# jedward225/MARL-HideAndSeek

Hardware: AMD Instinct MI355X
Metric: world-steps/sec (agent-steps/sec derived) at 16K worlds, 1/2/4/8 GPU (higher is better)
Workload: dtype f32; 1 GPU; 16000 worlds/GPU x 2646 steps, 2 hiders + 2 seekers, sim_flags=0, rand_seed=0, random move actions in [-5,4] each step (scripts/benchmark.py args); worlds_per_gpu=16000, total_worlds=16000, agents_per_world=4

## Files before the change

### marl-hideandseek_amd/csrc/hs_k_physics.h

```cpp
#pragma once
#include "hs_state.h"
#include "hs_rays.h"
#include "hs_collide.h"
#include "hs_solver.h"
#include "hs_broadphase.h"
#include "hs_k_reset.h"

namespace hs {

constexpr int kPhysThreads = 64;
constexpr int kWorldLanes = kPhysThreads / kTile;
constexpr int kLdsWalls = 32;
static_assert(kMaxSCand <= 32 && kMaxDDCand <= 16, "accepted-manifold masks are one word per world");
constexpr int kAllDD = kNumDSlots * (kNumDSlots - 1) / 2;
constexpr int kAllSC = kNumDSlots * (kMaxWalls + kMaxPlanes - 1);
constexpr int kSpInfoWords = kNumDSlots + 1;

struct alignas(16) OctRes {
    static constexpr int kClip = kClipLanes;
    static constexpr int kClipWords = clip_words(kClip);
    static constexpr int kSatPairs = kClip < hs::kSatPairs ? kClip : hs::kSatPairs;
    static constexpr int kMaxItems = kTile * (kMaxDDCand + kMaxSCand);
    static constexpr int kSlots = kClip < 31 ? kClip : 31;
    static constexpr int kVelOffsetWords = 2 * 8 * 3 * 32;
    float pos[3][kNumDSlots][kTile];
    float rot[4][kNumDSlots][kTile];
    float ppos[3][kNumDSlots][kTile];
    float prot[4][kNumDSlots][kTile];
    int meta[kNumDSlots][kTile];
    union {
        struct {
            float lo[3][kNumDSlots][kTile], hi[3][kNumDSlots][kTile];
            float wall[4][kLdsWalls][kTile];
            unsigned xch[kNumDSlots][kTile];
        } det;
        struct {
            float clip[kClipWords];
            unsigned short items[kMaxItems + 32];
            int pend[4][kClip];
        } sat;
        struct {
            float pad[kVelOffsetWords];
            float lin[3][kNumDSlots][kTile];
            float ang[3][kNumDSlots][kTile];
        } vel;
    } u;
    unsigned short ddPair[kMaxDDCand][kTile];
    unsigned short scPair[kMaxSCand][kTile];
    unsigned short scInfo[kNumDSlots][kTile];
    unsigned int scAcc[kTile];
    unsigned int ddAcc[kTile];
    unsigned int ddOrd[2][kTile];
    float plane0[4][kTile];
    unsigned char bodies[kNumDSlots * kTile];
    union {
        unsigned char wallBodies[kNumDSlots * kTile];
        unsigned char actGL[kMaxAgents][kTile];
    };
    unsigned int wallSeen[kTile];
    unsigned char numWalls[kTile], numPlanes[kTile], ndd[kTile], nsc[kTile], seen[kTile], hasGrab[kTile];
    unsigned char spill[kTile];
    int wid[kTile];
};
constexpr int kSeenDeferred = 2;
static_assert(sizeof(OctRes) <= 20 * 1024, "8 waves of 8 worlds share the CU's 160 KiB of LDS");
static_assert(offsetof(OctRes, u.sat.items) >= offsetof(OctRes, u.det.wall), "items must not overlap the AABBs");
static_assert(sizeof(decltype(OctRes::u.det)) <= sizeof(decltype(OctRes::u.sat)), "the broadphase scratch adds nothing to the octet's LDS");
static_assert(sizeof(ManDD) / 4 * OctRes::kSlots <= OctRes::kVelOffsetWords, "manifold slots lie below the velocities");
static_assert(2 * 3 * kNumDSlots * 8 <= OctRes::kVelOffsetWords, "the hull AABBs lie below the velocities");

constexpr int kLocGlobal = 31;
HSD int pair_a(int p) { return p & 31; }
HSD int pair_b(int p) { return (p >> 5) & 63; }
HSD int pair_loc(int p) { return (p >> 11) & 31; }
HSD int pair_pack(int a, int b) { return a | (b << 5) | (kLocGlobal << 11); }
static_assert(kNumDSlots <= 32 && kMaxWalls + kMaxPlanes <= 64, "pair encoding");
static_assert(sizeof(ManDD) % 16 == 0 && sizeof(ManS) % 16 == 0, "manifold records move 16 bytes at a time");
constexpr int kManWords = sizeof(ManDD) / 4;
template <typename M> HSD void man_lds_load(const float *clip, int slot, M &m) {
    m = *reinterpret_cast<const M *>(clip + slot * kManWords);
}
template <typename M> HSD void man_lds_set_lam(float *clip, int slot, int j, float v) {
    static_assert(offsetof(M, lam) == sizeof(M) - 16, "lam is the record's tail");
    clip[slot * kManWords + (sizeof(M) / 4 - 4 + j)] = v;
}

template <int C> HSD V3 rld3(const float (&a)[C][kNumDSlots][kTile], int slot, int g) { return {a[0][slot][g], a[1][slot][g], a[2][slot][g]}; }
HSD Q rld4(const float (&a)[4][kNumDSlots][kTile], int slot, int g) { return {a[0][slot][g], a[1][slot][g], a[2][slot][g], a[3][slot][g]}; }
HSD void rst3(float (&a)[3][kNumDSlots][kTile], int slot, int g, V3 v) { a[0][slot][g] = v.x; a[1][slot][g] = v.y; a[2][slot][g] = v.z; }
HSD void rst4(float (&a)[4][kNumDSlots][kTile], int slot, int g, Q q) { a[0][slot][g] = q.w; a[1][slot][g] = q.x; a[2][slot][g] = q.y; a[3][slot][g] = q.z; }

HSD void rbody_load(const OctRes &R, int g, int slot, BodyS &b) {
    b.pos = rld3(R.pos, slot, g); b.rot = rld4(R.rot, slot, g);
    b.ppos = rld3(R.ppos, slot, g); b.prot = rld4(R.prot, slot, g);
    b.lin = rld3(R.u.vel.lin, slot, g); b.ang = rld3(R.u.vel.ang, slot, g);
    const int m = R.meta[slot][g];
    const bool dyn = m != 0 && meta_resp(m) == RESP_DYNAMIC;
    b.invM = dyn ? obj_inv_mass(meta_obj(m)) : 0.f;
    b.invI = dyn ? obj_inv_inertia(meta_obj(m)) : V3{0.f, 0.f, 0.f};
    body_refresh_inertia(b);
}
HSD void rbody_store_pose(OctRes &R, int g, int slot, const BodyS &b) { rst3(R.pos, slot, g, b.pos); rst4(R.rot, slot, g, b.rot); }
HSD void rbody_store_vel(OctRes &R, int g, int slot, const BodyS &b) { rst3(R.u.vel.lin, slot, g, b.lin); rst3(R.u.vel.ang, slot, g, b.ang); }
HSD void derive_velocity(BodyS &b) {
    const float h = kSubstepH;
    b.lin = (b.pos - b.ppos) * (1.f / h);
    Q dq = qmul(b.rot, qinv(b.prot));
    V3 wv = V3{dq.x, dq.y, dq.z} * (2.f / h);
    b.ang = dq.w >= 0.f ? wv : -wv;
}

HSD void wave_sync() { asm volatile("s_waitcnt lgkmcnt(0)" ::: "memory"); }
HSD void mem_sync() { asm volatile("s_waitcnt vmcnt(0) lgkmcnt(0)" ::: "memory"); }

template <int D> HSD int dpp_row_shr(int x) { return __builtin_amdgcn_update_dpp(0, x, 0x110 + D, 0xF, 0xF, true); }
HSD int scan8_incl(int x, int l) {
    int y;
// ... 334 lines not shown
    if (l == 0) {
        R.spill[g] = (unsigned char)((spillDD ? 1 : 0) | (spillSC ? 2 : 0));
        if (spillDD || spillSC) spInfo[0] = tot_dd | (tot_sc << 16);
        R.ndd[g] = (unsigned char)min(tot_dd, kMaxDDCand); R.nsc[g] = (unsigned char)min(tot_sc, kMaxSCand);
        if (R.wid[g] >= 0 && tot_dd + tot_sc > 0) S.loadAcc[R.wid[g]] += tot_dd + tot_sc;
    }
    wave_sync();
    return ic;
}

template <bool POS, int UNROLL, typename SetLam>
HSD void static_manifold(BodyS &me, const ManS &m, SetLam set_lam) {
    BodyS none;
    body_refresh_inertia(me);
    const V3 n = ld3(m.n);
    const int np = m.np;
    const float mu = POS ? m.muS : m.muD;
#pragma unroll UNROLL
    for (int j = 0; j < 4; ++j)
        if (j < np) {
            const float lamj = m.lam[j];
            if (POS) set_lam(j, lamj + solve_point_position<false>(me, none, n, ld3(m.rA[j]), V3{0.f, 0.f, 0.f}, m.offB[j], mu));
            else solve_point_velocity<false>(me, none, n, ld3(m.rA[j]), V3{0.f, 0.f, 0.f}, lamj, mu);
        }
}

#define HS_COLD __device__ __forceinline__
struct SpillCtx {
    const float *walls, *planes;
    ManDD *wsDD; ManS *wsSC; unsigned short *spPair; int *spInfo;
    int wbeg;
};
HSD SpillCtx spill_ctx(const SimState &S) { return {S.walls.p, S.planes.p, (ManDD *)S.wsDD, (ManS *)S.wsSC, S.spPair, S.spInfo, S.wbeg}; }

HS_COLD void spill_sat(SpillCtx c, OctRes *Rp) {
    OctRes &R = *Rp;
    const int lane = hs_lane() & 63;
    const bool hi = (lane & 1) != 0;
    const Col<float, 4 * kMaxWalls> walls = {const_cast<float *>(c.walls)};
    const Col<float, 4 * kMaxPlanes> planes = {const_cast<float *>(c.planes)};
#pragma unroll 1
    for (int g = 0; g < kTile; ++g) {
        const int fl = __builtin_amdgcn_readfirstlane((int)R.spill[g]);
        if (fl == 0) continue;
        const int w = c.wbeg + g;
        const int tot = __builtin_amdgcn_readfirstlane(c.spInfo[(size_t)w * kSpInfoWords]);
#pragma unroll 1
        for (int kind = 0; kind < 2; ++kind) {
            if ((fl & (1 << kind)) == 0) continue;
            const bool isdd = kind == 0;
            const int n = isdd ? tot & 0xffff : tot >> 16;
#pragma unroll 1
            for (int base = isdd ? kMaxDDCand : kMaxSCand; base < n; base += OctRes::kSatPairs) {
                const int kk = base + (lane >> 1);
                if (kk < n && (lane >> 1) < OctRes::kSatPairs) {
                    const int pair = c.spPair[(size_t)w * (kAllDD + kAllSC) + (isdd ? 0 : kAllDD) + kk];
                    const int a = pair_a(pair), bsel = pair_b(pair);
                    const int oa = meta_obj(R.meta[a][g]);
                    const V3 pa = rld3(R.pos, a, g);
                    const Q qa = rld4(R.rot, a, g);
                    ManDD *const md = c.wsDD + (size_t)w * kAllDD + kk;
                    ManS *const ms = c.wsSC + (size_t)w * kAllSC + kk;
                    RawManifold raw;
                    raw.np = 0;
                    bool plane = false;
                    if (!isdd && bsel >= kMaxWalls) {
                        const int p = bsel - kMaxWalls;
                        const V3 pn = {planes(0 * kMaxPlanes + p, w), planes(1 * kMaxPlanes + p, w), planes(2 * kMaxPlanes + p, w)};
                        plane = true;
                        if (!hi && !collide_hull_plane(hull_ref_body(oa, pa, qa), pn, planes(3 * kMaxPlanes + p, w), raw)) raw.np = 0;
                    } else {
                        const HullSrc ha = hull_src_body(oa, pa, qa);
                        const HullSrc hb = isdd ? hull_src_body(meta_obj(R.meta[bsel][g]), rld3(R.pos, bsel, g), rld4(R.rot, bsel, g))
                                                : hull_src_wall(walls(0 * kMaxWalls + bsel, w), walls(1 * kMaxWalls + bsel, w),
                                                                walls(2 * kMaxWalls + bsel, w), walls(3 * kMaxWalls + bsel, w));
                        const AxisResult res = sat_axes(ha, hb, hi);
                        const ClipBuf cb = {R.u.sat.clip, lane >> 1, OctRes::kClip};
                        if (!hi && res.code != 0 && !sat_contact(ha, hb, res, cb, raw)) raw.np = 0;
                    }
                    if (!hi) {
                        const int ob = isdd ? meta_obj(R.meta[bsel][g]) : plane ? OBJ_PLANE : OBJ_WALL;
                        const float muS = 0.5f * (obj_mu_s(oa) + obj_mu_s(ob)), muD = 0.5f * (obj_mu_d(oa) + obj_mu_d(ob));
                        const Q qai = qinv(qa);
                        if (isdd) {
                            md->a = a; md->b = bsel; md->np = raw.np; md->muS = muS; md->muD = muD;
                            st3(md->n, raw.n);
                            const V3 pb = rld3(R.pos, bsel, g);
                            const Q qbi = qinv(rld4(R.rot, bsel, g));
#pragma unroll
                            for (int j = 0; j < 4; ++j)
                                if (j < raw.np) {
                                    st3(md->rA[j], qrot(qai, raw.pA[j] - pa)); st3(md->rB[j], qrot(qbi, raw.pB[j] - pb));
                                    md->lam[j] = 0.f;
                                }
                        } else {
                            ms->np = raw.np; ms->muS = muS; ms->muD = muD;
                            st3(ms->n, raw.n);
#pragma unroll
                            for (int j = 0; j < 4; ++j)
                                if (j < raw.np) {
                                    st3(ms->rA[j], plane ? hull_local_vertex(oa, raw.vidx[j]) : qrot(qai, raw.pA[j] - pa));
                                    ms->offB[j] = dot(raw.pB[j], raw.n); ms->lam[j] = 0.f;
                                }
                        }
                    }
                }
                wave_sync();
            }
// ... 30 lines not shown
                if (POS) { rbody_store_pose(R, g, ba, Ab); rbody_store_pose(R, g, bb, Bb); }
                else { rbody_store_vel(R, g, ba, Ab); rbody_store_vel(R, g, bb, Bb); }
                wave_sync();
            }
        }
    }
}

template <bool POS>
HS_COLD void spill_static(SpillCtx c, OctRes *Rp, int NS) {
    OctRes &R = *Rp;
#pragma unroll 1
    for (int g = 0; g < kTile; ++g) {
        if ((__builtin_amdgcn_readfirstlane((int)R.spill[g]) & 2) == 0) continue;
        const int w = c.wbeg + g;
        const int slot = hs_lane();
        if (slot >= NS) continue;
        const int info = c.spInfo[(size_t)w * kSpInfoWords + 1 + slot];
        const int first = info & 0xffff, cnt = info >> 16;
        if (cnt == 0) continue;
        BodyS me;
        rbody_load(R, g, slot, me);
#pragma unroll 1
        for (int k = first; k < first + cnt; ++k) {
            ManS &m = c.wsSC[(size_t)w * kAllSC + k];
            if (m.np <= 0) continue;
            static_manifold<POS, 1>(me, m, [&](int j, float v) { m.lam[j] = v; });
        }
        if (POS) rbody_store_pose(R, g, slot, me); else rbody_store_vel(R, g, slot, me);
    }
}

HSD HullSrc sat_hull_a(const OctRes &R, int g, int a) { return hull_src_body(meta_obj(R.meta[a][g]), rld3(R.pos, a, g), rld4(R.rot, a, g)); }
HSD HullSrc sat_hull_b(const SimState &S, const OctRes &R, int g, int w, bool isdd, int bsel) {
    if (isdd) return hull_src_body(meta_obj(R.meta[bsel][g]), rld3(R.pos, bsel, g), rld4(R.rot, bsel, g));
    return hull_src_wall(S.walls(0 * kMaxWalls + bsel, w), S.walls(1 * kMaxWalls + bsel, w),
                         S.walls(2 * kMaxWalls + bsel, w), S.walls(3 * kMaxWalls + bsel, w));
}
HSD bool sat_flush(const SimState &S, OctRes &R, int npend, bool last) {
    const int lane = hs_lane() & 63;
    const bool toLds = last && lane < OctRes::kSlots;
    bool wroteGlobal = false;
    int mw[kManWords]; int mkind = 0, mkk = 0, mg = 0, mpair = 0;
    if (lane < npend) {
        const int item = R.u.sat.pend[0][lane] & 0xffff;
        AxisResult res;
        res.code = R.u.sat.pend[0][lane] >> 16;
        res.ax = {__int_as_float(R.u.sat.pend[1][lane]), __int_as_float(R.u.sat.pend[2][lane]), __int_as_float(R.u.sat.pend[3][lane])};
        const int g = item >> 6, idx = item & 63;
        const int w = S.wbeg + g;
        const bool isdd = idx < 32;
        const int kk = idx & 31;
        const int pair = isdd ? R.ddPair[kk][g] : R.scPair[kk][g];
        const int a = pair_a(pair), bsel = pair_b(pair);
        const ClipBuf cb = {R.u.sat.clip, lane, OctRes::kClip};
        RawManifold raw;
        const bool plane = res.code == 3;
        bool have;
        if (plane) {
            const int p = bsel - kMaxWalls;
            const V3 pn = {S.planes(0 * kMaxPlanes + p, w), S.planes(1 * kMaxPlanes + p, w), S.planes(2 * kMaxPlanes + p, w)};
            have = collide_hull_plane(hull_ref_body(meta_obj(R.meta[a][g]), rld3(R.pos, a, g), rld4(R.rot, a, g)), pn, S.planes(3 * kMaxPlanes + p, w), raw);
        } else {
            have = sat_contact(sat_hull_a(R, g, a), sat_hull_b(S, R, g, w, isdd, bsel), res, cb, raw);
        }
        if (have) {
            const int oa = meta_obj(R.meta[a][g]);
            const int ob = isdd ? meta_obj(R.meta[bsel][g]) : plane ? OBJ_PLANE : OBJ_WALL;
            const V3 pa = rld3(R.pos, a, g);
            const Q qai = qinv(rld4(R.rot, a, g));
            const float muS = 0.5f * (obj_mu_s(oa) + obj_mu_s(ob)), muD = 0.5f * (obj_mu_d(oa) + obj_mu_d(ob));
            if (isdd) {
                ManDD m;
                m.a = a; m.b = bsel; m.np = raw.np; m.muS = muS; m.muD = muD;
                st3(m.n, raw.n);
                const V3 pb = rld3(R.pos, bsel, g);
                const Q qbi = qinv(rld4(R.rot, bsel, g));
#pragma unroll
                for (int j = 0; j < 4; ++j) {
                    const bool on = j < raw.np;
                    st3(m.rA[j], on ? qrot(qai, raw.pA[j] - pa) : V3{0.f, 0.f, 0.f});
                    st3(m.rB[j], on ? qrot(qbi, raw.pB[j] - pb) : V3{0.f, 0.f, 0.f});
                    m.lam[j] = 0.f;
                }
                if (toLds) { __builtin_memcpy(mw, &m, sizeof(m)); mkind = 1; mkk = kk; mg = g; mpair = pair; }
                else { ((ManDD *)S.wsDD + (size_t)w * kAllDD)[kk] = m; wroteGlobal = true; }
                atomicOr(&R.ddAcc[g], 1u << kk);
            } else {
                ManS m;
                m.np = raw.np; m.muS = muS; m.muD = muD; m.pad[0] = 0.f; m.pad[1] = 0.f;
                st3(m.n, raw.n);
#pragma unroll
                for (int j = 0; j < 4; ++j) {
                    const bool on = j < raw.np;
                    st3(m.rA[j], !on ? V3{0.f, 0.f, 0.f} : plane ? hull_local_vertex(oa, raw.vidx[j]) : qrot(qai, raw.pA[j] - pa));
                    m.offB[j] = on ? dot(raw.pB[j], raw.n) : 0.f; m.lam[j] = 0.f;
                }
// ... 22 lines not shown
HSD bool phase_sat(const SimState &S, OctRes &R, ItemCounts ic) {
    const int wedge0 = (ic.nbox + 31) / 32 * 32;
    const int lane = hs_lane() & 63;
    const bool hi = (lane & 1) != 0;
    int npend = 0;
    bool usedGlobal = false;
    const int boxRounds = (ic.nbox + OctRes::kSatPairs - 1) / OctRes::kSatPairs, wedgeRounds = (ic.nwedge + 3) / 4;
    if (__builtin_expect(ic.anySpill, 0)) { spill_sat(spill_ctx(S), &R); usedGlobal = true; }
    const int totalRounds = boxRounds + wedgeRounds;
    int round = 0;
    while (round < totalRounds) {
    for (; round < totalRounds; ++round) {
        const bool wide = round >= boxRounds;
        {
            const int itemsHere = wide ? min(4, wedge0 + ic.nwedge - (wedge0 + (round - boxRounds) * 4)) : min(OctRes::kSatPairs, ic.nbox - round * OctRes::kSatPairs);
            if (npend + itemsHere > OctRes::kClip) break;
        }
        const int base = wide ? wedge0 + (round - boxRounds) * 4 : round * OctRes::kSatPairs;
        const int it = wide ? base + (lane >> 4) : base + (lane >> 1);
        const bool lead = wide ? (lane & 15) == 0 : !hi;
        AxisResult res = {0, {0.f, 0.f, 0.f}};
        int item = 0;
        if (wide ? it < wedge0 + ic.nwedge : (it < ic.nbox && (lane >> 1) < OctRes::kSatPairs)) {
            item = R.u.sat.items[it];
            const int g = item >> 6, idx = item & 63;
            const int w = S.wbeg + g;
            const bool isdd = idx < 32;
            const int kk = idx & 31;
            const int pair = isdd ? R.ddPair[kk][g] : R.scPair[kk][g];
            const int a = pair_a(pair), bsel = pair_b(pair);
            if (!isdd && bsel >= kMaxWalls) {
                if (lead) res.code = 3;
            } else if (wide) {
                res = sat_axes_wide(sat_hull_a(R, g, a), sat_hull_b(S, R, g, w, isdd, bsel), lane & 15);
            } else {
                res = sat_axes(sat_hull_a(R, g, a), sat_hull_b(S, R, g, w, isdd, bsel), hi);
            }
        }
        const bool hit = lead && res.code != 0;
        const unsigned long long m = __ballot(hit);
        const int nhit = __popcll(m);
        if (hit) {
            const int pos = npend + __popcll(m & ((1ull << lane) - 1ull));
            R.u.sat.pend[0][pos] = item | (res.code << 16);
            R.u.sat.pend[1][pos] = __float_as_int(res.ax.x); R.u.sat.pend[2][pos] = __float_as_int(res.ax.y); R.u.sat.pend[3][pos] = __float_as_int(res.ax.z);
        }
        npend += nhit;
    }
    wave_sync();
    if (npend > 0) { usedGlobal |= sat_flush(S, R, npend, round >= totalRounds); npend = 0; }
    }
    if (usedGlobal) mem_sync();
    return usedGlobal;
}

HSD void solve_grab_joint_bodies(BodyS &A, BodyS &B, V3 r2, Q attach2, float sep, V3 r1, Q attach1) {
    {
        Q qa = qmul(A.rot, attach1), qb = qmul(B.rot, attach2);
        Q dq = qmul(qa, qinv(qb));
        V3 dphi = {2.f * dq.x, 2.f * dq.y, 2.f * dq.z};
        if (dq.w < 0.f) dphi = -dphi;
        float th2 = len2(dphi);
        if (th2 > 1e-12f) {
            float th = sqrtf(th2);
            V3 ax = dphi * (1.f / th);
            float wA = dot(ax, sym_mul(A.Iw, ax));
            float wB = dot(ax, sym_mul(B.Iw, ax));
            float ws = wA + wB;
            if (ws > 0.f) {
// ... 65 lines not shown
HSD void pair_point_velocity(BodyS &me, bool isA, V3 n, V3 rl, float lamN, float muD) {
    if (!(lamN > 0.f)) return;
    const V3 rw = qrot(me.rot, rl);
    const bool hm = me.invM + me.invI.x + me.invI.y + me.invI.z != 0.f;
    const V3 vm = cross_add(me.ang, rw, me.lin);
    const V3 vo = swap1(vm);
    const bool ho = swap1(hm ? 1.f : 0.f) != 0.f;
    const V3 vA = isA ? vm : vo, vB = isA ? vo : vm;
    const bool hA = isA ? hm : ho, hB = isA ? ho : hm;
    V3 v = {0.f, 0.f, 0.f};
    if (hA) v = vA;
    if (hB) v = v - vB;
    const float vn = dot(n, v);
    const V3 vt = nmadd(v, n, vn);
    const float vt2 = len2(vt);
    V3 dv = -(n * vn);
    if (vt2 > 1e-18f) {
        const float vtl = sqrtf(vt2);
        const float mag = fminf((muD * lamN) * kInvSubstepH, vtl);
        dv = nmadd(dv, vt, mag / vtl);
    }
    const float dv2 = len2(dv);
    if (!(dv2 > 1e-18f)) return;
    const float wm = gen_inv_mass_sq(me, rw, dv, dv2);
    const float wo = swap1(wm);
    const float ws = isA ? wm + wo : wo + wm;
    if (!(ws > 0.f)) return;
    const V3 p = dv * (dv2 / ws);
    const V3 da = apply_inv_inertia(me, cross(rw, p));
    if (isA) { me.lin = madd(me.lin, p, me.invM); me.ang = me.ang + da; }
    else { me.lin = nmadd(me.lin, p, me.invM); me.ang = me.ang - da; }
}

template <bool POS>
HSD void phase_dd(const SimState &S, OctRes &R, bool anySpill) {
    constexpr int GL = kWorldLanes, PAIRS = GL / 2;
    const int L = hs_lane(), g = L / GL, q = L % GL;
    const int h = q >> 1;
    const bool isA = (q & 1) == 0;
    const int gbit0 = g * GL;
    const int w = S.wbeg + g;
    const int ndd = R.ndd[g];
    const bool grab = R.hasGrab[g] != 0;
    if (!anySpill && __ballot(R.ddAcc[g] != 0u || (POS && grab)) == 0ull) return;
    if (POS && grab && q == 0) {
        const int teams = S.teams[R.wid[g]];
        for (int a = 0; a < kMaxAgents; ++a) {
            if (!team_agent_active(teams, a)) continue;
            const int other = S.grabOther(a, w);
            if (other < 0) continue;
            BodyS A, B;
            rbody_load(R, g, kAgentSlot0 + a, A); rbody_load(R, g, other, B);
            float gd[kGrabWords];
#pragma unroll
            for (int c = 0; c < kGrabWords; ++c) gd[c] = S.grabData(c * kMaxAgents + a, w);
            solve_grab_joint_bodies(A, B, {gd[0], gd[1], gd[2]}, {gd[3], gd[4], gd[5], gd[6]}, gd[7],
                                    {gd[8], gd[9], gd[10]}, {gd[11], gd[12], gd[13], gd[14]});
            rbody_store_pose(R, g, kAgentSlot0 + a, A); rbody_store_pose(R, g, other, B);
        }
    }
    ManDD *const wsDD = (ManDD *)S.wsDD + (size_t)w * kAllDD;
    const unsigned acc = R.ddAcc[g];
    const int nacc = __popc(acc);
    if (POS) {
        if (q < 2) R.ddOrd[q][g] = 0u;
        int key0 = 0x7fffffff, key1 = 0x7fffffff;
        if (q < ndd && ((acc >> q) & 1u)) { const int p = R.ddPair[q][g]; key0 = (pair_a(p) << 8) | pair_b(p); }
        if (q + GL < ndd && ((acc >> (q + GL)) & 1u)) { const int p = R.ddPair[q + GL][g]; key1 = (pair_a(p) << 8) | pair_b(p); }
        int rank0 = 0, rank1 = 0;
#pragma unroll
        for (int p = 0; p < GL; ++p) {
            const int k0 = __shfl(key0, gbit0 + p), k1 = __shfl(key1, gbit0 + p);
            rank0 += (k0 < key0) + (k1 < key0); rank1 += (k0 < key1) + (k1 < key1);
        }
        wave_sync();
        if (key0 != 0x7fffffff) atomicOr(&R.ddOrd[rank0 >> 3][g], (unsigned)q << ((rank0 & 7) * 4));
        if (key1 != 0x7fffffff) atomicOr(&R.ddOrd[rank1 >> 3][g], (unsigned)(q + GL) << ((rank1 & 7) * 4));
    }
    wave_sync();
    for (int base = 0; base < kMaxDDCand; base += PAIRS) {
        if (__ballot(base < nacc) == 0ull) break;
        const int rk = base + h;
        const int mine = rk < nacc ? (int)((R.ddOrd[rk >> 3][g] >> ((rk & 7) * 4)) & 15u) : -1;
        int ma = -1, mb = -1, loc = kLocGlobal;
        ManDD m;
        if (mine >= 0) {
            const int pr = R.ddPair[mine][g];
            ma = pair_a(pr); mb = pair_b(pr); loc = pair_loc(pr);
            if (loc != kLocGlobal) man_lds_load(R.u.sat.clip, loc, m); else m = wsDD[mine];
        }
        unsigned dep = 0u;
#pragma unroll
        for (int p = 0; p < PAIRS - 1; ++p) {
            const int pa = __shfl(ma, gbit0 + 2 * p), pb = __shfl(mb, gbit0 + 2 * p);
            if (p < h && pa >= 0 && (pa == ma || pa == mb || pb == ma || pb == mb)) dep |= 1u << p;
        }
        bool pending = mine >= 0;
        BodyS me;
        const int myBody = isA ? ma : mb;
        const V3 n = ld3(m.n);
        while (true) {
            const unsigned long long pend_mask = __ballot(pending && isA);
            if (pend_mask == 0ull) break;
            const unsigned wp = (unsigned)(pend_mask >> gbit0);
            unsigned pendPairs = 0u;
#pragma unroll
            for (int p = 0; p < PAIRS; ++p) pendPairs |= ((wp >> (2 * p)) & 1u) << p;
            if (pending && (dep & pendPairs) == 0u) {
                rbody_load(R, g, myBody, me);
                if (POS) {
#pragma unroll
                    for (int j = 0; j < 4; ++j)
                        if (j < m.np) {
                            const float lam = pair_point_position(me, isA, n, isA ? ld3(m.rA[j]) : ld3(m.rB[j]), m.muS);
                            if (isA) { if (loc != kLocGlobal) man_lds_set_lam<ManDD>(R.u.sat.clip, loc, j, m.lam[j] + lam); else wsDD[mine].lam[j] = m.lam[j] + lam; }
                        }
                    rbody_store_pose(R, g, myBody, me);
                } else {
#pragma unroll
                    for (int j = 0; j < 4; ++j)
                        if (j < m.np) pair_point_velocity(me, isA, n, isA ? ld3(m.rA[j]) : ld3(m.rB[j]), m.lam[j], m.muD);
                    rbody_store_vel(R, g, myBody, me);
                }
                pending = false;
            }
            wave_sync();
        }
    }
    wave_sync();
    if (__builtin_expect(anySpill, 0)) { spill_dd<POS>(spill_ctx(S), &R); wave_sync(); }
}

struct WallLists { int nwb, nEarly; };
template <int ROUNDS>
HSD WallLists list_wall_bodies(OctRes &R, int nbodies, int lastRound) {
    const int L = hs_lane();
    int n = 0, nEarly = 0;
#pragma unroll
    for (int r = 0; r < ROUNDS; ++r) {
        if (r == lastRound) nEarly = n;
        const bool valid = r * 64 + L < nbodies;
        const int t = valid ? R.bodies[r * 64 + L] : 0;
        const int sci = valid ? R.scInfo[t >> 3][t & 7] : 0;
        const bool on = sci != 0 && ((R.scAcc[t & 7] >> (sci & 0xff)) & ((1u << (sci >> 8)) - 1u)) != 0u;
        const unsigned long long m = __ballot(on);
        if (on) { R.wallBodies[n + __popcll(m & ((1ull << L) - 1ull))] = (unsigned char)t; atomicOr(&R.wallSeen[t & 7], 1u << (t >> 3)); }
        n += __popcll(m);
    }
    wave_sync();
    return {n, nEarly};
}

HSD void ground_pos(OctRes &R, BodyReg &b, int slot, int g, int meta) {
    if (meta_resp(meta) != RESP_DYNAMIC || b.np == 0) return;
    const int obj = meta_obj(meta);
    BodyS me;
    rbody_load(R, g, slot, me);
    const V3 gn = -V3{R.plane0[0][g], R.plane0[1][g], R.plane0[2][g]};
    const float gmuS = 0.5f * (obj_mu_s(obj) + obj_mu_s(OBJ_PLANE));
    const bool yaw = slot >= kAgentSlot0;
    float dj[4] = {0.f, 0.f, 0.f, 0.f}, share = 0.f;
    if (yaw) share = yaw_ground_prepass(me, gn, b.np, hull_local_vertex(obj, b.vidx & 7), hull_local_vertex(obj, (b.vidx >> 3) & 7),
                                        hull_local_vertex(obj, (b.vidx >> 6) & 7), hull_local_vertex(obj, (b.vidx >> 9) & 7), kGroundOff, dj);
// ... 4 lines not shown
    rbody_store_pose(R, g, slot, me);
}
HSD void ground_vel(OctRes &R, const BodyReg &b, int slot, int g, int meta) {
    if (meta_resp(meta) != RESP_DYNAMIC || b.np == 0) return;
    const int obj = meta_obj(meta);
    BodyS me, none;
    rbody_load(R, g, slot, me);
    const V3 gn = -V3{R.plane0[0][g], R.plane0[1][g], R.plane0[2][g]};
    const float gmuD = 0.5f * (obj_mu_d(obj) + obj_mu_d(OBJ_PLANE));
#pragma unroll
    for (int j = 0; j < 4; ++j)
        if (j < b.np) solve_point_velocity<false>(me, none, gn, hull_local_vertex(obj, (b.vidx >> (3 * j)) & 7), V3{0.f, 0.f, 0.f},
                                                  b.lam[j], gmuD);
    rbody_store_vel(R, g, slot, me);
}
template <bool POS>
HSD void wall_round(const SimState &S, OctRes &R, int first, int nwb) {
    for (int i = first + hs_lane(); i < nwb; i += 64) {
        const int t = R.wallBodies[i];
        const int slot = t >> 3, g = t & 7;
        const int sci = R.scInfo[slot][g];
        const int bsc = sci & 0xff, asc = sci >> 8;
        const unsigned acc = R.scAcc[g];
        ManS *const wsSC = (ManS *)S.wsSC + (size_t)(S.wbeg + g) * kAllSC;
        BodyS me;
        rbody_load(R, g, slot, me);
        unsigned todo = (acc >> bsc) & ((1u << asc) - 1u);
#pragma unroll 1
        while (todo != 0u) {
            const int k = bsc + __ffs((int)todo) - 1;
            todo &= todo - 1u;
            const int loc = pair_loc(R.scPair[k][g]);
            ManS m;
            if (loc != kLocGlobal) man_lds_load(R.u.sat.clip, loc, m); else m = wsSC[k];
            static_manifold<POS, 4>(me, m, [&](int j, float v) {
                if (loc != kLocGlobal) man_lds_set_lam<ManS>(R.u.sat.clip, loc, j, v); else wsSC[k].lam[j] = v;
            });
        }
        if (POS) rbody_store_pose(R, g, slot, me); else rbody_store_vel(R, g, slot, me);
    }
}
template <bool POS>
HSD void last_round(const SimState &S, OctRes &R, BodyReg &b, bool valid, int slot, int g, int meta, int nLast, int nMerged) {
    const int mi = (int)hs_lane() - nLast;
    const bool walls = mi >= 0 && mi < nMerged;
    unsigned todo = 0u; int bsc = 0;
    if (walls) {
        const int t = R.wallBodies[mi];
        slot = t >> 3; g = t & 7; meta = R.meta[slot][g];
        const int sci = R.scInfo[slot][g];
        bsc = sci & 0xff;
        todo = (R.scAcc[g] >> bsc) & ((1u << (sci >> 8)) - 1u);
    } else if (valid && meta_resp(meta) == RESP_DYNAMIC && b.np != 0) {
        todo = 1u;
    }
    if (todo == 0u) return;
    const int obj = meta_obj(meta);
    BodyS me, none;
    rbody_load(R, g, slot, me);
    ManS *const wsSC = (ManS *)S.wsSC + (size_t)(S.wbeg + g) * kAllSC;
#pragma unroll 1
    while (todo != 0u) {
        const int k = bsc + __ffs((int)todo) - 1;
        todo &= todo - 1u;
        V3 n; float mu; int np, loc = kLocGlobal;
        ManS m;
        if (walls) {
            loc = pair_loc(R.scPair[k][g]);
            if (loc != kLocGlobal) man_lds_load(R.u.sat.clip, loc, m); else m = wsSC[k];
            n = ld3(m.n); mu = POS ? m.muS : m.muD; np = m.np;
        } else {
            n = -V3{R.plane0[0][g], R.plane0[1][g], R.plane0[2][g]};
            mu = POS ? 0.5f * (obj_mu_s(obj) + obj_mu_s(OBJ_PLANE)) : 0.5f * (obj_mu_d(obj) + obj_mu_d(OBJ_PLANE));
            np = b.np;
        }
        body_refresh_inertia(me);
        const bool yaw = POS && !walls && slot >= kAgentSlot0;
        float dj[4] = {0.f, 0.f, 0.f, 0.f}, share = 0.f;
        if (yaw) share = yaw_ground_prepass(me, n, np, hull_local_vertex(obj, b.vidx & 7), hull_local_vertex(obj, (b.vidx >> 3) & 7),
                                            hull_local_vertex(obj, (b.vidx >> 6) & 7), hull_local_vertex(obj, (b.vidx >> 9) & 7), kGroundOff, dj);
#define HS_LAST_POINT(j)                                                                                                   \
        if ((j) < np) {                                                                                                    \
            const V3 rAj = walls ? ld3(m.rA[j]) : hull_local_vertex(obj, (b.vidx >> (3 * (j))) & 7);                       \
            const float lamj = walls ? m.lam[j] : b.lam[j];                                                                \
            if (POS) {                                                                                                     \
                const float nl = lamj + solve_point_position_ground(me, n, rAj, walls ? m.offB[j] : kGroundOff, mu, yaw, dj[j], share); \
                if (!walls) b.lam[j] = nl;                                                                                 \
                else if (loc != kLocGlobal) man_lds_set_lam<ManS>(R.u.sat.clip, loc, (j), nl);                             \
                else wsSC[k].lam[j] = nl;                                                                                  \
            } else {                                                                                                       \
                solve_point_velocity<false>(me, none, n, rAj, V3{0.f, 0.f, 0.f}, lamj, mu);                                \
            }                                                                                                              \
        }
        HS_LAST_POINT(0) HS_LAST_POINT(1) HS_LAST_POINT(2) HS_LAST_POINT(3)
#undef HS_LAST_POINT
    }
    if (POS) rbody_store_pose(R, g, slot, me); else rbody_store_vel(R, g, slot, me);
}
HSD void derive_body_velocity(OctRes &R, int slot, int g, int meta) {
    if (meta_resp(meta) != RESP_DYNAMIC) return;
    BodyS me;
    me.pos = rld3(R.pos, slot, g); me.rot = rld4(R.rot, slot, g);
    me.ppos = rld3(R.ppos, slot, g); me.prot = rld4(R.prot, slot, g);
    derive_velocity(me);
    rbody_store_vel(R, g, slot, me);
}

HSD void action_system(const SimState &S, OctRes &R, int g, int A_, int teams) {
    const int w = S.wbeg + g;
    const ResGeom geom = {R, S, g, w};
    for (int i = 0; i < A_; ++i) {
        const int fl = R.actGL[i][g];
        if (fl == 0) continue;
        const int type = team_agent_type(teams, i);
        const int slot = kAgentSlot0 + i;
        const V3 mpos = geom.g_pos(slot);
        const Q mrot = geom.g_rot(slot);
        if (fl & 2) {
            float t; V3 o = mpos + V3{0.f, 0.f, 0.5f};
            int hit = trace_ray(geom, o, qrot(mrot, {0.f, 1.f, 0.f}), 2.5f, &t);
            if (hit >= 0 && hit < kNumDSlots) {
                const int m = R.meta[hit][g];
                const int obj = meta_obj(m), resp = meta_resp(m), owner = meta_owner(m);
                if (resp == RESP_STATIC) {
                    if ((type == AGENT_SEEKER && owner == OWNER_SEEKER) || (type == AGENT_HIDER && owner == OWNER_HIDER))
                        R.meta[hit][g] = meta_pack(obj, RESP_DYNAMIC, OWNER_NONE);
                } else if (owner == OWNER_NONE) {
                    R.meta[hit][g] = meta_pack(obj, RESP_STATIC, type == AGENT_HIDER ? OWNER_HIDER : OWNER_SEEKER);
// ... 151 lines not shown
    const int L = hs_lane();
#pragma unroll
    for (int r = 0; r < LASTR; ++r) {
        const bool valid = r * 64 + L < nbodies; const int t_ = valid ? R.bodies[r * 64 + L] : 0;
        const int slot = t_ >> 3, g = t_ & 7; const int meta = valid ? R.meta[slot][g] : 0;
        if (valid) { if (POS) ground_pos(R, br[r], slot, g, meta); else ground_vel(R, br[r], slot, g, meta); }
    }
    wave_sync();
    {
        const bool valid = LASTR * 64 + L < nbodies; const int t_ = valid ? R.bodies[LASTR * 64 + L] : 0;
        const int slot = t_ >> 3, g = t_ & 7; const int meta = valid ? R.meta[slot][g] : 0;
        last_round<POS>(S, R, br[LASTR], valid, slot, g, meta, nLast, nMerged);
    }
    wave_sync();
}

#ifdef HS_PHASE_TIMING
#define HS_TICK_PARAMS , long long &tk, long long (&acc)[10]
#define HS_TICK_ARGS , tk, acc
#define HS_TICK(i) { const long long now_ = wall_clock64(); acc[i] += now_ - tk; tk = now_; }
#else
#define HS_TICK_PARAMS
#define HS_TICK_ARGS
#define HS_TICK(i)
#endif
#define HS_BODY(r) const bool valid = (r) * 64 + L < nbodies; const int t_ = valid ? R.bodies[(r) * 64 + L] : 0; \
                   const int slot = t_ >> 3, g = t_ & 7; const int meta = valid ? R.meta[slot][g] : 0;
template <int ROUNDS>
HSD void substep_rest(const SimState &S, OctRes &R, BodyReg (&br)[ROUNDS], int nbodies, int NS, ItemCounts ic, bool integrateNext,
                      const float *aforce HS_TICK_PARAMS) {
    const int L = hs_lane();
    const bool manGlobal = phase_sat(S, R, ic);
    HS_TICK(3)
    phase_dd<true>(S, R, ic.anySpill);
    HS_TICK(4)
    constexpr int kShortLastR = ROUNDS - 2;
    const bool shortLast = ROUNDS == 3 && nbodies <= 64 * (ROUNDS - 1);
    const int lastRound = shortLast ? kShortLastR : ROUNDS - 1;
    const WallLists wl = list_wall_bodies<ROUNDS>(R, nbodies, lastRound);
    const int nLast = max(nbodies - 64 * lastRound, 0);
    const int nMerged = min(wl.nEarly, 64 - nLast);
    if (shortLast) static_passes<ROUNDS, kShortLastR, true>(S, R, br, nbodies, nLast, nMerged);
    else static_passes<ROUNDS, ROUNDS - 1, true>(S, R, br, nbodies, nLast, nMerged);
    if (wl.nwb > nMerged) { wall_round<true>(S, R, nMerged, wl.nwb); wave_sync(); }
    if (__builtin_expect(ic.anySpill, 0)) { spill_static<true>(spill_ctx(S), &R, NS); wave_sync(); }
#pragma unroll
    for (int r = 0; r < ROUNDS; ++r) { HS_BODY(r) if (valid) derive_body_velocity(R, slot, g, meta); }
    if (manGlobal) mem_sync(); else wave_sync();
    HS_TICK(5)
    phase_dd<false>(S, R, ic.anySpill);
    HS_TICK(6)
    if (shortLast) static_passes<ROUNDS, kShortLastR, false>(S, R, br, nbodies, nLast, nMerged);
    else static_passes<ROUNDS, ROUNDS - 1, false>(S, R, br, nbodies, nLast, nMerged);
    if (wl.nwb > nMerged) { wall_round<false>(S, R, nMerged, wl.nwb); wave_sync(); }
    if (__builtin_expect(ic.anySpill, 0)) { spill_static<false>(spill_ctx(S), &R, NS); wave_sync(); }
    if (integrateNext) {
#pragma unroll
        for (int r = 0; r < ROUNDS; ++r) { HS_BODY(r) if (valid) integrate_body(R, br[r], slot, g, meta, aforce); }
        wave_sync();
    }
    HS_TICK(7)
}

template <int ROUNDS>
HSD void physics_step(SimState &S, OctRes &R, GenScratch *gen) {
    const int L = hs_lane();
    const int noct = gridDim.x;
    const int sidx = step_ring(S), prevIdx = sidx == 0 ? 2 : sidx - 1, nextIdx = sidx == 2 ? 0 : sidx + 1;
    const int serve = step_serve(S);
    if (serve != kGroupEarly && blockIdx.x == 0 && L == 0) {
        S.tickSum[nextIdx] = 0ull;
        atomicExch(group_count(S, prevIdx, kGroupEarly), 0); atomicExch(group_count(S, prevIdx, kGroupLate), 0);
    }
    int o = blockIdx.x;
    if (serve != kGroupAll) {
        if (o >= *group_count(S, sidx, serve)) return;
        o = oct_list(S, sidx, serve, noct)[o];
    }
    S.wbeg = o * kTile;
    const int p0 = S.wbeg;
    const int NS = kAgentSlot0 + S.A;
    const long long tStart = wall_clock64();
    int prevTicks, lateAbove;
// ... 117 lines not shown
```

Measured before the change: 35.20 million world-steps/s.

## Carry body-pair solve order in registers and load only each side's manifold pieces

```diff
diff --git a/marl-hideandseek_amd/csrc/hs_k_physics.h b/marl-hideandseek_amd/csrc/hs_k_physics.h
--- a/marl-hideandseek_amd/csrc/hs_k_physics.h
+++ b/marl-hideandseek_amd/csrc/hs_k_physics.h
@@ -4,6 +4,7 @@
 #include "hs_collide.h"
 #include "hs_solver.h"
 #include "hs_broadphase.h"
+#include "hs_solve_order.h"
 #include "hs_k_reset.h"
 
 namespace hs {
@@ -50,7 +51,6 @@
     unsigned short scInfo[kNumDSlots][kTile];
     unsigned int scAcc[kTile];
     unsigned int ddAcc[kTile];
-    unsigned int ddOrd[2][kTile];
     float plane0[4][kTile];
     unsigned char bodies[kNumDSlots * kTile];
     union {
@@ -77,12 +77,31 @@
 static_assert(kNumDSlots <= 32 && kMaxWalls + kMaxPlanes <= 64, "pair encoding");
 static_assert(sizeof(ManDD) % 16 == 0 && sizeof(ManS) % 16 == 0, "manifold records move 16 bytes at a time");
 constexpr int kManWords = sizeof(ManDD) / 4;
-template <typename M> HSD void man_lds_load(const float *clip, int slot, M &m) {
-    m = *reinterpret_cast<const M *>(clip + slot * kManWords);
-}
-template <typename M> HSD void man_lds_set_lam(float *clip, int slot, int j, float v) {
+typedef float Piece __attribute__((ext_vector_type(4)));
+#define HS_LDS __attribute__((address_space(3)))
+#define HS_GLOBAL __attribute__((address_space(1)))
+HSD Piece lds_piece(const float *p) { return *(const HS_LDS Piece *)p; }
+HSD Piece glb_piece(const float *p) { return *(const HS_GLOBAL Piece *)p; }
+HSD void lds_put_piece(float *p, Piece v) { *(HS_LDS Piece *)p = v; }
+HSD void glb_put_piece(float *p, Piece v) { *(HS_GLOBAL Piece *)p = v; }
+HSD float glb_word(const float *p) { return *(const HS_GLOBAL float *)p; }
+template <int N> struct Pieces { Piece p[N]; };
+template <int N> HSD void man_load(const float *clip, int loc, const float *rec, const int (&at)[N], Pieces<N> &out) {
+    const float *s = clip + min(loc, OctRes::kSlots - 1) * kManWords;
+#pragma unroll
+    for (int i = 0; i < N; ++i) out.p[i] = lds_piece(s + at[i]);
+    if (loc == kLocGlobal) {
+#pragma unroll
+        for (int i = 0; i < N; ++i) out.p[i] = glb_piece(rec + at[i]);
+    }
+}
+template <typename M> HSD void man_put_lam(float *clip, int loc, M *rec, Piece lam) {
     static_assert(offsetof(M, lam) == sizeof(M) - 16, "lam is the record's tail");
-    clip[slot * kManWords + (sizeof(M) / 4 - 4 + j)] = v;
+    if (loc != kLocGlobal) lds_put_piece(clip + loc * kManWords + (sizeof(M) / 4 - 4), lam);
+    else glb_put_piece(rec->lam, lam);
+}
+HSD void man_static_load(const float *clip, int loc, const ManS *rec, ManS &m) {
+    if (loc != kLocGlobal) m = *reinterpret_cast<const ManS *>(clip + loc * kManWords); else m = *rec;
 }
 
 template <int C> HSD V3 rld3(const float (&a)[C][kNumDSlots][kTile], int slot, int g) { return {a[0][slot][g], a[1][slot][g], a[2][slot][g]}; }
@@ -483,6 +502,7 @@
     int wbeg;
 };
 HSD SpillCtx spill_ctx(const SimState &S) { return {S.walls.p, S.planes.p, (ManDD *)S.wsDD, (ManS *)S.wsSC, S.spPair, S.spInfo, S.wbeg}; }
+HSD HullSrc sat_hull_b(const Col<float, 4 * kMaxWalls> &walls, const OctRes &R, int g, int w, bool isdd, int bsel);
 
 HS_COLD void spill_sat(SpillCtx c, OctRes *Rp) {
     OctRes &R = *Rp;
@@ -522,9 +542,7 @@
                         if (!hi && !collide_hull_plane(hull_ref_body(oa, pa, qa), pn, planes(3 * kMaxPlanes + p, w), raw)) raw.np = 0;
                     } else {
                         const HullSrc ha = hull_src_body(oa, pa, qa);
-                        const HullSrc hb = isdd ? hull_src_body(meta_obj(R.meta[bsel][g]), rld3(R.pos, bsel, g), rld4(R.rot, bsel, g))
-                                                : hull_src_wall(walls(0 * kMaxWalls + bsel, w), walls(1 * kMaxWalls + bsel, w),
-                                                                walls(2 * kMaxWalls + bsel, w), walls(3 * kMaxWalls + bsel, w));
+                        const HullSrc hb = sat_hull_b(walls, R, g, w, isdd, bsel);
                         const AxisResult res = sat_axes(ha, hb, hi);
                         const ClipBuf cb = {R.u.sat.clip, lane >> 1, OctRes::kClip};
                         if (!hi && res.code != 0 && !sat_contact(ha, hb, res, cb, raw)) raw.np = 0;
@@ -621,10 +639,14 @@
 }
 
 HSD HullSrc sat_hull_a(const OctRes &R, int g, int a) { return hull_src_body(meta_obj(R.meta[a][g]), rld3(R.pos, a, g), rld4(R.rot, a, g)); }
-HSD HullSrc sat_hull_b(const SimState &S, const OctRes &R, int g, int w, bool isdd, int bsel) {
-    if (isdd) return hull_src_body(meta_obj(R.meta[bsel][g]), rld3(R.pos, bsel, g), rld4(R.rot, bsel, g));
-    return hull_src_wall(S.walls(0 * kMaxWalls + bsel, w), S.walls(1 * kMaxWalls + bsel, w),
-                         S.walls(2 * kMaxWalls + bsel, w), S.walls(3 * kMaxWalls + bsel, w));
+HSD HullSrc sat_hull_b(const Col<float, 4 * kMaxWalls> &walls, const OctRes &R, int g, int w, bool isdd, int bsel) {
+    static_assert(kNumDSlots <= kMaxWalls, "a body slot is a valid wall row");
+    const float *const wp = &walls(min(bsel, kMaxWalls - 1), w);
+    const float cx = glb_word(wp), cy = glb_word(wp + kMaxWalls * kTile);
+    const float hx = glb_word(wp + 2 * kMaxWalls * kTile), hy = glb_word(wp + 3 * kMaxWalls * kTile);
+    const int slot = isdd ? bsel : 0;
+    const HullSrc body = hull_src_body(meta_obj(R.meta[slot][g]), rld3(R.pos, slot, g), rld4(R.rot, slot, g));
+    return hull_src_sel(isdd, body, hull_src_wall(cx, cy, hx, hy));
 }
 HSD bool sat_flush(const SimState &S, OctRes &R, int npend, bool last) {
     const int lane = hs_lane() & 63;
@@ -651,7 +673,7 @@
             const V3 pn = {S.planes(0 * kMaxPlanes + p, w), S.planes(1 * kMaxPlanes + p, w), S.planes(2 * kMaxPlanes + p, w)};
             have = collide_hull_plane(hull_ref_body(meta_obj(R.meta[a][g]), rld3(R.pos, a, g), rld4(R.rot, a, g)), pn, S.planes(3 * kMaxPlanes + p, w), raw);
         } else {
-            have = sat_contact(sat_hull_a(R, g, a), sat_hull_b(S, R, g, w, isdd, bsel), res, cb, raw);
+            have = sat_contact(sat_hull_a(R, g, a), sat_hull_b(S.walls, R, g, w, isdd, bsel), res, cb, raw);
         }
         if (have) {
             const int oa = meta_obj(R.meta[a][g]);
@@ -740,9 +762,9 @@
             if (!isdd && bsel >= kMaxWalls) {
                 if (lead) res.code = 3;
             } else if (wide) {
-                res = sat_axes_wide(sat_hull_a(R, g, a), sat_hull_b(S, R, g, w, isdd, bsel), lane & 15);
+                res = sat_axes_wide(sat_hull_a(R, g, a), sat_hull_b(S.walls, R, g, w, isdd, bsel), lane & 15);
             } else {
-                res = sat_axes(sat_hull_a(R, g, a), sat_hull_b(S, R, g, w, isdd, bsel), hi);
+                res = sat_axes(sat_hull_a(R, g, a), sat_hull_b(S.walls, R, g, w, isdd, bsel), hi);
             }
         }
         const bool hit = lead && res.code != 0;
@@ -874,17 +896,32 @@
     else { me.lin = nmadd(me.lin, p, me.invM); me.ang = me.ang - da; }
 }
 
+struct ManSide { int np; float muS, muD; V3 n; V3 r[4]; Piece lam; };
+HSD void man_side_load(const float *clip, int loc, const ManDD *rec, bool isA, ManSide &m) {
+    static_assert(offsetof(ManDD, rA) == 32 && offsetof(ManDD, rB) == 80 && offsetof(ManDD, lam) == 128, "pieces of a ManDD");
+    const int r0 = isA ? 8 : 20;
+    const int at[6] = {0, 4, r0, r0 + 4, r0 + 8, 32};
+    Pieces<6> q;
+    man_load(clip, loc, reinterpret_cast<const float *>(rec), at, q);
+    m.np = __float_as_int(q.p[0].z); m.muS = q.p[0].w; m.muD = q.p[1].x;
+    m.n = {q.p[1].y, q.p[1].z, q.p[1].w};
+    m.r[0] = {q.p[2].x, q.p[2].y, q.p[2].z}; m.r[1] = {q.p[2].w, q.p[3].x, q.p[3].y};
+    m.r[2] = {q.p[3].z, q.p[3].w, q.p[4].x}; m.r[3] = {q.p[4].y, q.p[4].z, q.p[4].w};
+    m.lam = q.p[5];
+}
+
 template <bool POS>
-HSD void phase_dd(const SimState &S, OctRes &R, bool anySpill) {
+HSD unsigned phase_dd(const SimState &S, OctRes &R, bool anySpill, unsigned ordIn) {
     constexpr int GL = kWorldLanes, PAIRS = GL / 2;
+    static_assert(PAIRS == kOrdBatch && kMaxDDCand <= kOrdBatch * kOrdBatches, "the order word holds every batch");
     const int L = hs_lane(), g = L / GL, q = L % GL;
     const int h = q >> 1;
     const bool isA = (q & 1) == 0;
     const int gbit0 = g * GL;
     const int w = S.wbeg + g;
-    const int ndd = R.ndd[g];
     const bool grab = R.hasGrab[g] != 0;
-    if (!anySpill && __ballot(R.ddAcc[g] != 0u || (POS && grab)) == 0ull) return;
+    const unsigned acc = R.ddAcc[g];
+    if (!anySpill && __ballot(acc != 0u || (POS && grab)) == 0ull) return 0u;
     if (POS && grab && q == 0) {
         const int teams = S.teams[R.wid[g]];
         for (int a = 0; a < kMaxAgents; ++a) {
@@ -902,66 +939,47 @@
         }
     }
     ManDD *const wsDD = (ManDD *)S.wsDD + (size_t)w * kAllDD;
-    const unsigned acc = R.ddAcc[g];
     const int nacc = __popc(acc);
-    if (POS) {
-        if (q < 2) R.ddOrd[q][g] = 0u;
-        int key0 = 0x7fffffff, key1 = 0x7fffffff;
-        if (q < ndd && ((acc >> q) & 1u)) { const int p = R.ddPair[q][g]; key0 = (pair_a(p) << 8) | pair_b(p); }
-        if (q + GL < ndd && ((acc >> (q + GL)) & 1u)) { const int p = R.ddPair[q + GL][g]; key1 = (pair_a(p) << 8) | pair_b(p); }
-        int rank0 = 0, rank1 = 0;
-#pragma unroll
-        for (int p = 0; p < GL; ++p) {
-            const int k0 = __shfl(key0, gbit0 + p), k1 = __shfl(key1, gbit0 + p);
-            rank0 += (k0 < key0) + (k1 < key0); rank1 += (k0 < key1) + (k1 < key1);
-        }
-        wave_sync();
-        if (key0 != 0x7fffffff) atomicOr(&R.ddOrd[rank0 >> 3][g], (unsigned)q << ((rank0 & 7) * 4));
-        if (key1 != 0x7fffffff) atomicOr(&R.ddOrd[rank1 >> 3][g], (unsigned)(q + GL) << ((rank1 & 7) * 4));
-    }
-    wave_sync();
-    for (int base = 0; base < kMaxDDCand; base += PAIRS) {
+    unsigned ord = POS ? 0u : ordIn;
+    wave_sync();
+    for (int base = 0, batch = 0; base < kMaxDDCand; base += PAIRS, ++batch) {
         if (__ballot(base < nacc) == 0ull) break;
         const int rk = base + h;
-        const int mine = rk < nacc ? (int)((R.ddOrd[rk >> 3][g] >> ((rk & 7) * 4)) & 15u) : -1;
-        int ma = -1, mb = -1, loc = kLocGlobal;
-        ManDD m;
+        const int mine = POS ? (rk < nacc ? kth_set_bit(acc, rk) : -1) : ord_cand(ord, batch);
+        int code = -1, loc = kLocGlobal;
+        ManSide m;
         if (mine >= 0) {
             const int pr = R.ddPair[mine][g];
-            ma = pair_a(pr); mb = pair_b(pr); loc = pair_loc(pr);
-            if (loc != kLocGlobal) man_lds_load(R.u.sat.clip, loc, m); else m = wsDD[mine];
-        }
-        unsigned dep = 0u;
-#pragma unroll
-        for (int p = 0; p < PAIRS - 1; ++p) {
-            const int pa = __shfl(ma, gbit0 + 2 * p), pb = __shfl(mb, gbit0 + 2 * p);
-            if (p < h && pa >= 0 && (pa == ma || pa == mb || pb == ma || pb == mb)) dep |= 1u << p;
-        }
+            code = pr & 0x7ff; loc = pair_loc(pr);
+            man_side_load(R.u.sat.clip, loc, wsDD + mine, isA, m);
+        }
+        unsigned dep;
+        if (POS) {
+            dep = batch_dep_mask(h, code, dpp_row_shr<2>(code), dpp_row_shr<4>(code), dpp_row_shr<6>(code));
+            if (mine >= 0) ord |= ord_pack(batch, mine, dep);
+        } else {
+            dep = ord_dep(ord, batch);
+        }
+        const unsigned depBits = dep_spread(dep);
         bool pending = mine >= 0;
         BodyS me;
-        const int myBody = isA ? ma : mb;
-        const V3 n = ld3(m.n);
+        const int myBody = isA ? pair_a(code) : pair_b(code);
         while (true) {
             const unsigned long long pend_mask = __ballot(pending && isA);
             if (pend_mask == 0ull) break;
-            const unsigned wp = (unsigned)(pend_mask >> gbit0);
-            unsigned pendPairs = 0u;
-#pragma unroll
-            for (int p = 0; p < PAIRS; ++p) pendPairs |= ((wp >> (2 * p)) & 1u) << p;
-            if (pending && (dep & pendPairs) == 0u) {
+            if (pending && (depBits & (unsigned)(pend_mask >> gbit0)) == 0u) {
                 rbody_load(R, g, myBody, me);
                 if (POS) {
+                    Piece lam = m.lam;
 #pragma unroll
                     for (int j = 0; j < 4; ++j)
-                        if (j < m.np) {
-                            const float lam = pair_point_position(me, isA, n, isA ? ld3(m.rA[j]) : ld3(m.rB[j]), m.muS);
-                            if (isA) { if (loc != kLocGlobal) man_lds_set_lam<ManDD>(R.u.sat.clip, loc, j, m.lam[j] + lam); else wsDD[mine].lam[j] = m.lam[j] + lam; }
-                        }
+                        if (j < m.np) lam[j] = lam[j] + pair_point_position(me, isA, m.n, m.r[j], m.muS);
+                    if (isA) man_put_lam(R.u.sat.clip, loc, wsDD + mine, lam);
                     rbody_store_pose(R, g, myBody, me);
                 } else {
 #pragma unroll
                     for (int j = 0; j < 4; ++j)
-                        if (j < m.np) pair_point_velocity(me, isA, n, isA ? ld3(m.rA[j]) : ld3(m.rB[j]), m.lam[j], m.muD);
+                        if (j < m.np) pair_point_velocity(me, isA, m.n, m.r[j], m.lam[j], m.muD);
                     rbody_store_vel(R, g, myBody, me);
                 }
                 pending = false;
@@ -971,6 +989,7 @@
     }
     wave_sync();
     if (__builtin_expect(anySpill, 0)) { spill_dd<POS>(spill_ctx(S), &R); wave_sync(); }
+    return ord;
 }
 
 struct WallLists { int nwb, nEarly; };
@@ -1041,10 +1060,10 @@
             todo &= todo - 1u;
             const int loc = pair_loc(R.scPair[k][g]);
             ManS m;
-            if (loc != kLocGlobal) man_lds_load(R.u.sat.clip, loc, m); else m = wsSC[k];
-            static_manifold<POS, 4>(me, m, [&](int j, float v) {
-                if (loc != kLocGlobal) man_lds_set_lam<ManS>(R.u.sat.clip, loc, j, v); else wsSC[k].lam[j] = v;
-            });
+            man_static_load(R.u.sat.clip, loc, wsSC + k, m);
+            Piece lam = {m.lam[0], m.lam[1], m.lam[2], m.lam[3]};
+            static_manifold<POS, 4>(me, m, [&](int j, float v) { lam[j] = v; });
+            if (POS) man_put_lam(R.u.sat.clip, loc, wsSC + k, lam);
         }
         if (POS) rbody_store_pose(R, g, slot, me); else rbody_store_vel(R, g, slot, me);
     }
@@ -1076,7 +1095,7 @@
         ManS m;
         if (walls) {
             loc = pair_loc(R.scPair[k][g]);
-            if (loc != kLocGlobal) man_lds_load(R.u.sat.clip, loc, m); else m = wsSC[k];
+            man_static_load(R.u.sat.clip, loc, wsSC + k, m);
             n = ld3(m.n); mu = POS ? m.muS : m.muD; np = m.np;
         } else {
             n = -V3{R.plane0[0][g], R.plane0[1][g], R.plane0[2][g]};
@@ -1094,15 +1113,14 @@
             const float lamj = walls ? m.lam[j] : b.lam[j];                                                                \
             if (POS) {                                                                                                     \
                 const float nl = lamj + solve_point_position_ground(me, n, rAj, walls ? m.offB[j] : kGroundOff, mu, yaw, dj[j], share); \
-                if (!walls) b.lam[j] = nl;                                                                                 \
-                else if (loc != kLocGlobal) man_lds_set_lam<ManS>(R.u.sat.clip, loc, (j), nl);                             \
-                else wsSC[k].lam[j] = nl;                                                                                  \
+                if (!walls) b.lam[j] = nl; else m.lam[j] = nl;                                                             \
             } else {                                                                                                       \
                 solve_point_velocity<false>(me, none, n, rAj, V3{0.f, 0.f, 0.f}, lamj, mu);                                \
             }                                                                                                              \
         }
         HS_LAST_POINT(0) HS_LAST_POINT(1) HS_LAST_POINT(2) HS_LAST_POINT(3)
 #undef HS_LAST_POINT
+        if (POS && walls) man_put_lam(R.u.sat.clip, loc, wsSC + k, Piece{m.lam[0], m.lam[1], m.lam[2], m.lam[3]});
     }
     if (POS) rbody_store_pose(R, g, slot, me); else rbody_store_vel(R, g, slot, me);
 }
@@ -1320,7 +1338,7 @@
     const int L = hs_lane();
     const bool manGlobal = phase_sat(S, R, ic);
     HS_TICK(3)
-    phase_dd<true>(S, R, ic.anySpill);
+    const unsigned ddOrder = phase_dd<true>(S, R, ic.anySpill, 0u);
     HS_TICK(4)
     constexpr int kShortLastR = ROUNDS - 2;
     const bool shortLast = ROUNDS == 3 && nbodies <= 64 * (ROUNDS - 1);
@@ -1336,7 +1354,7 @@
     for (int r = 0; r < ROUNDS; ++r) { HS_BODY(r) if (valid) derive_body_velocity(R, slot, g, meta); }
     if (manGlobal) mem_sync(); else wave_sync();
     HS_TICK(5)
-    phase_dd<false>(S, R, ic.anySpill);
+    phase_dd<false>(S, R, ic.anySpill, ddOrder);
     HS_TICK(6)
     if (shortLast) static_passes<ROUNDS, kShortLastR, false>(S, R, br, nbodies, nLast, nMerged);
     else static_passes<ROUNDS, ROUNDS - 1, false>(S, R, br, nbodies, nLast, nMerged);
diff --git a/marl-hideandseek_amd/csrc/hs_solve_order.h b/marl-hideandseek_amd/csrc/hs_solve_order.h
--- /dev/null
+++ b/marl-hideandseek_amd/csrc/hs_solve_order.h
@@ -0,0 +1,40 @@
+#pragma once
+#include "hs_core.h"
+
+namespace hs {
+
+constexpr int kOrdBatch = 4;
+constexpr int kOrdBatches = 4;
+
+HSD int kth_set_bit(unsigned mask, int k) {
+    int pos = 0;
+    int c = __builtin_popcount(mask & 0xffu);
+    if (k >= c) { k -= c; pos += 8; mask >>= 8; }
+    c = __builtin_popcount(mask & 0xfu);
+    if (k >= c) { k -= c; pos += 4; mask >>= 4; }
+    c = __builtin_popcount(mask & 0x3u);
+    if (k >= c) { k -= c; pos += 2; mask >>= 2; }
+    c = (int)(mask & 1u);
+    if (k >= c) pos += 1;
+    return pos;
+}
+
+HSD bool pairs_touch(int x, int y) {
+    const int xa = x & 31, xb = (x >> 5) & 63, ya = y & 31, yb = (y >> 5) & 63;
+    return (xa == ya) | (xa == yb) | (xb == ya) | (xb == yb);
+}
+HSD unsigned batch_dep_mask(int h, int mine, int prev1, int prev2, int prev3) {
+    unsigned dep = 0u;
+    if (mine < 0) return dep;
+    if (h >= 1 && prev1 >= 0 && pairs_touch(mine, prev1)) dep |= 1u << (h - 1);
+    if (h >= 2 && prev2 >= 0 && pairs_touch(mine, prev2)) dep |= 1u << (h - 2);
+    if (h >= 3 && prev3 >= 0 && pairs_touch(mine, prev3)) dep |= 1u << (h - 3);
+    return dep;
+}
+
+HSD unsigned ord_pack(int batch, int cand, unsigned dep) { return ((unsigned)cand | 16u | (dep << 5)) << (8 * batch); }
+HSD int ord_cand(unsigned ord, int batch) { const unsigned b = ord >> (8 * batch); return (b & 16u) ? (int)(b & 15u) : -1; }
+HSD unsigned ord_dep(unsigned ord, int batch) { return (ord >> (8 * batch + 5)) & 7u; }
+HSD unsigned dep_spread(unsigned dep) { return (dep & 1u) | ((dep & 2u) << 1) | ((dep & 4u) << 2); }
+
+}
```

Result: faster. 35.58 million world-steps/s, median of 6 (+1.1%).
